# kezakool/flair-for-aigle

Hardware: AMD Instinct MI355X
Metric: 512x512x5 tiles/sec (train fwd+bwd+AdamW), U-Net ResNet-34, 19 classes (higher is better)
Workload: dtype bf16; 1 GPU; synthetic 512x512x5 tiles, 19-class U-Net (ResNet-34 encoder), batch 32 per GPU, train step (BASELINE.json configs[1]); global_batch=32, tile=512, parallelism=dp1

## Files before the change

flair-for-aigle_amd/csrc/conv_igemm.hip:

```cpp
#include "ffa_gfx950.h"

#include <stdlib.h>

#ifndef FFA_CONV_READS_FIRST
#define FFA_CONV_READS_FIRST 0
#endif

#ifndef FFA_CONV_TRACE
#define FFA_CONV_TRACE 0
#endif
#if FFA_CONV_TRACE
#ifndef FFA_CONV_TRACE_FIRST
#define FFA_CONV_TRACE_FIRST 0
#endif
__device__ long long ffa_conv_trace_buf[64 * 256];
#define FFA_TRACE(slot_)                                                                    \
  if (trace_on) {                                                                           \
    if (trace_n < 256) ffa_conv_trace_buf[(blockIdx.x - FFA_CONV_TRACE_FIRST) * 256 + trace_n] = (long long)(slot_) << 56 | (__builtin_readcyclecounter() & 0xFFFFFFFFFFFFFFLL); \
    ++trace_n;                                                                              \
  }
#else
#define FFA_TRACE(slot_)
#endif

// ... 867 lines not shown
            }
            if (res) {
#pragma unroll
              for (int i = 0; i < 4; ++i) v[i] += ffa_load_elem<T>(res + pix + c0 + i);
            }
            if (a.relu) {
#pragma unroll
              for (int i = 0; i < 4; ++i) v[i] = fmaxf(v[i], 0.f);
            }
            if (EB == 2) {
              uint2 u;
              u.x = ffa_pack_bf16x2(v[0], v[1]);
              u.y = ffa_pack_bf16x2(v[2], v[3]);
              *reinterpret_cast<uint2*>(out + pix + c0) = u;
            } else {
              *reinterpret_cast<float4*>(out + pix + c0) = make_float4(v[0], v[1], v[2], v[3]);
            }
            if (want_stats) {
#pragma unroll
              for (int i = 0; i < 4; ++i) {
                const float r = (EB == 2) ? ffa_bf16_bits_to_f32(ffa_f32_to_bf16_bits(v[i])) : v[i];
                st[g * 4 + i] += r;
                st[NCH + g * 4 + i] = __builtin_fmaf(r, r, st[NCH + g * 4 + i]);
              }
            }
          }
        }
      }
      if (want_stats) {
#pragma unroll
        for (int bit = 4; bit >= 0; --bit) {
          const int n = (2 * NCH) >> (4 - bit);
          if (n > 2) {
            const bool up = (rho >> bit) & 1;
#pragma unroll
            for (int jj = 0; jj < NCH; ++jj) {
              if (jj < n / 2) {
                float lo = st[jj], hi = st[jj + n / 2];
                asm volatile("" : "+v"(lo), "+v"(hi));
                const float keep = up ? hi : lo;
                const float send = up ? lo : hi;
                st[jj] = keep + __shfl_xor(send, 1 << bit, 64);
              }
            }
          } else {
            st[0] += __shfl_xor(st[0], 1 << bit, 64);
            st[1] += __shfl_xor(st[1], 1 << bit, 64);
          }
        }
        red[(wpx * 64 + lane) * 2 + 0] = st[0];
        red[(wpx * 64 + lane) * 2 + 1] = st[1];
        __syncthreads();
        constexpr int NOUT = (G::MT == 2) ? 128 : 64;
        if (tid < NOUT) {
          const int jj = tid & 1;
          const int ln = (G::MT == 2) ? (tid >> 1) : ((tid >> 1) * 2);
          float t = 0.f;
#pragma unroll
          for (int w = 0; w < WPX; ++w) t += red[(w * 64 + ln) * 2 + jj];
          const int r5 = ln & 31, hf = ln >> 5;
          const int which = r5 >> 4;
          int c;
          if (G::MT == 2) {
            const int L = (r5 & 15) * 2 + jj;
            c = cur.cb * BCO + 16 * (L >> 3) + 8 * hf + (L & 7);
          } else {
            const int L = ((r5 >> 1) & 7) * 2 + jj;
            c = cur.cb * BCO + 8 * (L >> 2) + 4 * hf + (L & 3);
          }
          if (c < a.Co) a.stats[((size_t)cur.pt * 2 + which) * a.Co + c] = t;
        }
        __syncthreads();
      }
    }
    if (!has_next) break;
    vb = nvb;
    cur = nxt;
    w_b = w_n;
  }
#undef FFA_P_STORE_W
#undef FFA_P_STORE_H
}


struct ConvPlan {
  int bco;
  int rg;
  int th, tw;
};

static int conv_rg(int kh) { return kh == 7 ? 1 : kh; }

static int conv_pref_bco(int kh, int kw, int stride, int cout) {
  if (kh == 3 && kw == 3 && stride == 1) return cout > 32 ? 64 : 32;
  return cout > 32 ? 64 : 32;
}

static bool conv_supported(int kh, int kw, int stride, int bco) {
  const bool shape = (kh == 3 && kw == 3 && (stride == 1 || stride == 2)) ||
                     (kh == 1 && kw == 1 && (stride == 1 || stride == 2)) || (kh == 7 && kw == 7 && stride == 2);
  if (!shape) return false;
  return bco == 64 || bco == 32;
}

static int conv_persist_grid(int dil, int c1_out, const void* bnx, int grid) {
  const char* pe = getenv("FFA_CONV_PERSIST");
  if ((pe && pe[0] == '0') || dil != 1 || c1_out != 0 || bnx != nullptr) return 0;
  const char* pm = getenv("FFA_CONV_PERSIST_MIN");
  const char* pg = getenv("FFA_CONV_PERSIST_GRID");
  const int min_grid = pm ? atoi(pm) : 0;
  int pgrid = pg ? atoi(pg) : 512;
  pgrid = pgrid < 8 ? 8 : (pgrid / 8) * 8;
  if (grid <= min_grid) return 0;
  return pgrid < grid ? pgrid : grid;
}

template <typename T, int KH, int KW, int STRIDE, int RG, int BCO, int WCO, int WPX, int TH, int TW, int HK,
          bool UP = false>
static int launch_hk(const ConvArgs& a, hipStream_t stream) {
  const int grid = ffa_cdiv(a.npt, 8) * 8 * a.ncb;
  if constexpr (KH == 3 && KW == 3 && STRIDE == 1 && HK >= 2 && !UP && WCO == 1 && WPX == 4) {
    const int pgrid = conv_persist_grid(a.dil, a.c1_out, a.bnx, grid);
    if (pgrid > 0) {
      hipLaunchKernelGGL((conv3x3_persist_kernel<T, BCO, TH, TW, HK>), dim3(pgrid), dim3(256), 0, stream, a);
      return ffa_check_launch("conv3x3_persist");
    }
  }
  hipLaunchKernelGGL((conv_igemm_kernel<T, KH, KW, STRIDE, RG, BCO, WCO, WPX, TH, TW, HK, UP>), dim3(grid),
                     dim3(64 * WCO * WPX), 0, stream, a);
  return ffa_check_launch("conv_igemm");
}

template <typename T, int BCO, int TH, int TW>
static int launch_up(const ConvArgs& a, hipStream_t stream) {
  if (a.nchunks % 4 == 0) return launch_hk<T, 3, 3, 1, 3, BCO, 1, 4, TH, TW, 4, true>(a, stream);
  return launch_hk<T, 3, 3, 1, 3, BCO, 1, 4, TH, TW, 2, true>(a, stream);
}

template <typename T, int KH, int KW, int STRIDE, int RG, int BCO, int WCO, int WPX, int TH, int TW>
static int launch_cfg(const ConvArgs& a, hipStream_t stream) {
  if constexpr (KH == 3 && STRIDE == 1) {
    if (a.nchunks % 4 == 0) return launch_hk<T, KH, KW, STRIDE, RG, BCO, WCO, WPX, TH, TW, 4>(a, stream);
    if (a.nchunks % 2 == 0) return launch_hk<T, KH, KW, STRIDE, RG, BCO, WCO, WPX, TH, TW, 2>(a, stream);
  }
  return launch_hk<T, KH, KW, STRIDE, RG, BCO, WCO, WPX, TH, TW, 1>(a, stream);
}

template <typename T, int KH, int KW, int STRIDE, int RG>
static int launch_shape(const ConvArgs& a, const ConvPlan& p, hipStream_t stream) {
  const bool wide = (p.tw == 32);
#define FFA_CONV_CASE(BCO_, WCO_, WPX_)                                                      \
  if (p.bco == BCO_) {                                                                       \
    return wide ? launch_cfg<T, KH, KW, STRIDE, RG, BCO_, WCO_, WPX_, 8, 32>(a, stream)      \
                : launch_cfg<T, KH, KW, STRIDE, RG, BCO_, WCO_, WPX_, 16, 16>(a, stream);    \
  }
  FFA_CONV_CASE(64, 1, 4)
  FFA_CONV_CASE(32, 1, 4)
#undef FFA_CONV_CASE
  ffa_set_error("conv: no kernel for bco=%d", p.bco);
  return FFA_ERR_UNSUPPORTED;
}

template <typename T>
static int launch_dtype(const ConvArgs& a, int kh, int kw, int stride, const ConvPlan& p, hipStream_t stream) {
  if (kh == 3 && kw == 3 && stride == 1) return launch_shape<T, 3, 3, 1, 3>(a, p, stream);
  if (kh == 3 && kw == 3 && stride == 2) return launch_shape<T, 3, 3, 2, 3>(a, p, stream);
// ... 23 lines not shown
      return (cout <= 16 ? 16 : 32) | FFA_BCO_THIN | (ci_pitch == 32 ? FFA_BCO_THIN32 : 0);
  }
  allow_ring &= 1;
  const char* e = getenv("FFA_RING");
  const int eb = (dtype == FFA_BF16) ? 2 : 4;
  const bool on = (dtype == FFA_BF16) ? !(e && e[0] == '0') : (e && e[0] == '1');
  if (allow_ring && on && kh == 3 && kw == 3 && stride == 1 && cout >= 64 && (ci_pitch * eb) % 64 == 0)
    return 64 | FFA_BCO_RING;
  return bco;
}

extern "C" int ffa_conv_row_group(int kh) { return conv_rg(kh); }

static int conv2d_impl(int dtype, const void* in, const void* w_packed, const float* bias, const void* residual,
                       void* out, float* stat_partials, int B, int Hi, int Wi, int Ci, int Ho, int Wo, int Co,
                       int co_rows, int bco, int kh, int kw, int stride, int pad, int dil, int relu,
                       hipStream_t stream, void* out2 = nullptr, int c1_out = 0, const void* bnx = nullptr,
                       const float* bn_sc = nullptr, const float* bn_sh = nullptr) {
  FFA_REQUIRE(dtype == FFA_BF16 || dtype == FFA_F32, "conv: bad dtype %d", dtype);
  FFA_REQUIRE(in && w_packed && out, "conv: null pointer");
  FFA_REQUIRE(B > 0 && Hi > 0 && Wi > 0 && Ho > 0 && Wo > 0, "conv: bad dims");
  FFA_REQUIRE(Ci % 16 == 0 && Co % 8 == 0, "conv: channel pitch must be a multiple of 16 (in) / 8 (out), got %d/%d", Ci, Co);
  FFA_REQUIRE(dil == 1 || dil == 2, "conv: dil must be 1 or 2");
  FFA_REQUIRE(dil == 1 || stride == 1, "conv: zero-insertion input needs stride 1");
  FFA_REQUIRE((long long)B * Hi * Wi * Ci * (dtype == FFA_BF16 ? 2 : 4) < (1LL << 31),
              "conv: input tensor must be smaller than 2 GiB (32-bit piece offsets)");
  if (bco & FFA_BCO_STEM) {
    FFA_REQUIRE(dtype == FFA_BF16 && kh == 7 && kw == 7 && stride == 2 && pad == 3 && dil == 1 && c1_out == 0 && bnx == nullptr &&
                    residual == nullptr,
                "conv: a stem-layout operand serves the bf16 7x7 stride-2 pad-3 convolution only (no residual input)");
    return ffa_stem_conv7x7(in, w_packed, bias, out, stat_partials, B, Hi, Wi, Ci, Ho, Wo, Co, relu, stream);
  }
  if (bco & FFA_BCO_THIN) {
    FFA_REQUIRE(dtype == FFA_BF16 && kh == 3 && kw == 3 && stride == 1 && pad == 1 && dil == 1 && Hi == Ho && Wi == Wo &&
                    bnx == nullptr,
                "conv: a thin-layout operand serves bf16 3x3 stride-1 pad-1 convolutions only");
    if (c1_out > 0) {
      FFA_REQUIRE(c1_out == Co && out2 == nullptr && !stat_partials, "conv: thin pooled form takes C2 = 0 only");
      return ffa_thin_conv3x3(in, w_packed, nullptr, nullptr, out, nullptr, B, Hi, Wi, Ci, Co, co_rows, 0, 0, 1, stream);
    }
    return ffa_thin_conv3x3(in, w_packed, bias, residual, out, stat_partials, B, Hi, Wi, Ci, Co, co_rows, relu, 0, 0,
                            stream);
  }
  if (bco & FFA_BCO_RING) {
    FFA_REQUIRE(kh == 3 && kw == 3 && stride == 1 && pad == 1 && dil == 1 && Hi == Ho && Wi == Wo && c1_out == 0 &&
                    bnx == nullptr,
                "conv: a ring-layout operand serves plain 3x3 stride-1 pad-1 convolutions only");
    return ffa_ring_conv3x3(dtype, in, w_packed, bias, residual, out, stat_partials, nullptr, nullptr, B, Hi, Wi, Ci, Co,
                            co_rows, relu, stream);
  }
  if (!conv_supported(kh, kw, stride, bco)) {
    ffa_set_error("conv: unsupported kernel %dx%d stride %d block %d", kh, kw, stride, bco);
    return FFA_ERR_UNSUPPORTED;
  }
  ConvPlan p;
  p.bco = bco;
  p.rg = conv_rg(kh);
  p.tw = (Wo >= 32) ? 32 : 16;
  p.th = (Wo >= 32) ? 8 : 16;
  FFA_REQUIRE(co_rows % p.bco == 0, "conv: packed weight rows %d not a multiple of block %d", co_rows, p.bco);
  ConvArgs a;
  a.in = in;
  a.w = w_packed;
  a.out = out;
  a.bias = bias;
  a.stats = stat_partials;
  a.in2 = nullptr;
  a.c1_bytes = 0;
  a.out2 = out2;
  a.c1_out = c1_out;
  a.bnx = bnx;
  a.bn_sc = bn_sc;
  a.bn_sh = bn_sh;
  a.res = residual;
  a.B = B; a.Hi = Hi; a.Wi = Wi; a.Ci = Ci;
  a.Ho = Ho; a.Wo = Wo; a.Co = Co;
  a.pad = pad; a.dil = dil; a.relu = relu;
  const int eb = (dtype == FFA_BF16) ? 2 : 4;
  a.nchunks = Ci * eb / 32;
  a.tiles_x = ffa_cdiv(Wo, p.tw);
  a.tiles_y = ffa_cdiv(Ho, p.th);
  a.npt = B * a.tiles_x * a.tiles_y;
  a.ncb = co_rows / p.bco;
  if (dtype == FFA_BF16) return launch_dtype<ffa_bf16>(a, kh, kw, stride, p, stream);
  return launch_dtype<float>(a, kh, kw, stride, p, stream);
}

extern "C" int ffa_conv2d(int dtype, const void* in, const void* w_packed, const float* bias, const void* residual,
                          void* out, int B, int Hi, int Wi, int Ci, int Ho, int Wo, int Co, int co_rows, int bco,
                          int kh, int kw, int stride, int pad, int dil, int relu, hipStream_t stream) {
  return conv2d_impl(dtype, in, w_packed, bias, residual, out, nullptr, B, Hi, Wi, Ci, Ho, Wo, Co, co_rows, bco, kh, kw,
                     stride, pad, dil, relu, stream);
}

extern "C" int ffa_conv2d_pro(int dtype, const void* in, const void* w_packed, const float* bias, const void* residual,
                              void* out, float* stat_partials, const float* pro_scale, const float* pro_shift, int B,
                              int H, int W, int Ci, int Co, int co_rows, int bco, int relu, int up, hipStream_t stream) {
  FFA_REQUIRE(dtype == FFA_BF16 && in && w_packed && out && pro_scale && pro_shift, "conv_pro: bad arguments");
  if (bco & FFA_BCO_THIN)
    return ffa_thin_conv3x3_pro(in, w_packed, bias, residual, out, stat_partials, pro_scale, pro_shift, B, H, W, Ci, Co,
                                co_rows, relu, up, 0, stream);
  if ((bco & FFA_BCO_RING) && !up)
    return ffa_ring_conv3x3(dtype, in, w_packed, bias, residual, out, stat_partials, pro_scale, pro_shift, B, H, W, Ci, Co,
                            co_rows, relu, stream);
  ffa_set_error("conv_pro: no prologue kernel for this operand layout (bco 0x%x, up %d)", bco, up);
  return FFA_ERR_UNSUPPORTED;
}

extern "C" int ffa_conv2d_bnbwd(int dtype, const void* in, const void* w_packed, const void* residual, void* out,
                                float* stat_partials, const void* bnx, const float* bn_scale, const float* bn_shift,
                                int B, int Hi, int Wi, int Ci, int Ho, int Wo, int Co, int co_rows, int bco, int kh,
                                int kw, int stride, int pad, int dil, hipStream_t stream) {
  FFA_REQUIRE(stat_partials && bnx && bn_scale && bn_shift, "conv_bnbwd: null pointer");
  return conv2d_impl(dtype, in, w_packed, nullptr, residual, out, stat_partials, B, Hi, Wi, Ci, Ho, Wo, Co, co_rows,
                     bco, kh, kw, stride, pad, dil, 0, stream, nullptr, 0, bnx, bn_scale, bn_shift);
}

static long long conv_stat_rows_igemm(int B, int Ho, int Wo) {
  const int tw = (Wo >= 32) ? 32 : 16, th = (Wo >= 32) ? 8 : 16;
  return (long long)B * ffa_cdiv(Wo, tw) * ffa_cdiv(Ho, th);
}
extern "C" long long ffa_conv_stat_rows(int B, int Ho, int Wo, int co_rows, int bco) {
  if (bco & FFA_BCO_STEM) return ffa_stem_stat_rows(B, Ho, Wo);
  if (bco & FFA_BCO_THIN) return ffa_thin_stat_rows(B, Ho, Wo, (bco & FFA_BCO_THIN32) ? 32 : 16);
  if (bco & FFA_BCO_RING) return ffa_ring_stat_rows(B, Ho, Wo, co_rows);
  return conv_stat_rows_igemm(B, Ho, Wo);
}

extern "C" int ffa_conv_is_persistent(int dtype, int B, int Ho, int Wo, int Ci, int co_rows, int bco, int kh, int kw,
                                      int stride, int dil) {
  if (!(kh == 3 && kw == 3 && stride == 1) || bco <= 0 || co_rows % bco != 0) return 0;
  const int nchunks = Ci * (dtype == FFA_BF16 ? 2 : 4) / 32;
  if (nchunks % 2 != 0) return 0;
  if (bco & (FFA_BCO_RING | FFA_BCO_THIN | FFA_BCO_STEM)) return 0;
  const int npt = (int)conv_stat_rows_igemm(B, Ho, Wo);
  return conv_persist_grid(dil, 0, nullptr, ffa_cdiv(npt, 8) * 8 * (co_rows / bco)) > 0 ? 1 : 0;
}

extern "C" int ffa_conv2d_stats(int dtype, const void* in, const void* w_packed, const float* bias,
                                const void* residual, void* out, float* stat_partials, int B, int Hi, int Wi, int Ci,
                                int Ho, int Wo, int Co, int co_rows, int bco, int kh, int kw, int stride, int pad,
                                int dil, int relu, hipStream_t stream) {
  FFA_REQUIRE(stat_partials, "conv_stats: null statistics buffer");
  return conv2d_impl(dtype, in, w_packed, bias, residual, out, stat_partials, B, Hi, Wi, Ci, Ho, Wo, Co, co_rows, bco,
                     kh, kw, stride, pad, dil, relu, stream);
}

extern "C" int ffa_conv2d_upcat(int dtype, const void* lo, const void* skip, const void* w_packed, const float* bias,
                                void* out, float* stat_partials, int B, int Hl, int Wl, int C1, int C2, int Co,
                                int co_rows, int bco, int relu, hipStream_t stream) {
  FFA_REQUIRE(dtype == FFA_BF16 || dtype == FFA_F32, "conv_upcat: bad dtype %d", dtype);
  FFA_REQUIRE(lo && w_packed && out && (skip || C2 == 0), "conv_upcat: null pointer");
  FFA_REQUIRE(B > 0 && Hl > 0 && Wl > 0 && C1 > 0 && C2 >= 0 && C1 % 16 == 0 && C2 % 16 == 0 && Co % 8 == 0,
              "conv_upcat: bad dims");
  const int eb = (dtype == FFA_BF16) ? 2 : 4;
  const int Hi = 2 * Hl, Wi = 2 * Wl, Ci = C1 + C2;
  if (bco & FFA_BCO_THIN) {
    if (C2 != 0 || dtype != FFA_BF16) {
      ffa_set_error("conv_upcat: a thin-layout operand takes the skip-less form only");
      return FFA_ERR_UNSUPPORTED;
    }
    return ffa_thin_conv3x3(lo, w_packed, bias, nullptr, out, stat_partials, B, Hi, Wi, C1, Co, co_rows, relu, 1, 0, stream);
  }
  FFA_REQUIRE((long long)B * Hi * Wi * (C1 > C2 ? C1 : C2) * eb < (1LL << 31),
              "conv_upcat: source tensors must be smaller than 2 GiB (32-bit piece offsets)");
  if (!conv_supported(3, 3, 1, bco) || co_rows % bco != 0) {
// ... 72 lines not shown
```

flair-for-aigle_amd/csrc/conv_wgrad.hip:

```cpp
#include "ffa_gfx950.h"

#include <stdlib.h>

#ifndef FFA_WGRAD_TRACE
#define FFA_WGRAD_TRACE 0
#endif
#if FFA_WGRAD_TRACE
__device__ long long ffa_wgrad_trace_buf[64 * 256];
#define FFA_WTRACE(slot_)                                                                   \
  if (trace_on) {                                                                           \
    if (trace_n < 256)                                                                      \
      ffa_wgrad_trace_buf[(blockIdx.y * gridDim.x + blockIdx.x) * 256 + trace_n] =          \
          (long long)(slot_) << 56 | (__builtin_readcyclecounter() & 0xFFFFFFFFFFFFFFLL);    \
    ++trace_n;                                                                              \
  }
#else
#define FFA_WTRACE(slot_)
#endif

struct WgradArgs {
  const void* x;
  const void* dy;
  float* slabs;
  int B, Hi, Wi, Ci;
  int Ho, Wo, Co;
  int pad;
  int tiles_x, tiles_y, npt;
  int ncob, ncib, nsplit;
  const void* x2;
  int C1;
  int CoT, CiT;
  const float* pro_sc;
  const float* pro_sh;
  int ci_real;
};

template <int KH, int KW, int STRIDE, int RG, int WCO, int WCI, int WK, int TH, int TW, int EB>
struct WgradGeom {
  static constexpr int NTHR = 64 * WCO * WCI * WK;
  static constexpr int NPX = TH * TW;
  static constexpr bool ONE = (KH == 1 && KW == 1);
  static constexpr int LS = ONE ? 1 : STRIDE;
  static constexpr int GSTEP = ONE ? STRIDE : 1;
  static constexpr int NRG = KH / RG;
  static constexpr int IH = (TH - 1) * LS + RG;
  static constexpr int IW = (TW - 1) * LS + KW;
  static constexpr int TAPS = RG * KW;
  static constexpr int ROWB = 32 * EB;
  static constexpr int PARTS = ROWB / 16;
  static constexpr int DY_BYTES = WCO * NPX * ROWB;
  static constexpr int IN_BYTES = WCI * IH * IW * ROWB;
  static constexpr int STAGE_BYTES = DY_BYTES + IN_BYTES;
  static constexpr bool MERGE = (WK > 1) && (WCO * WCI == 4 || KH == 7);
  static constexpr int MERGE_BYTES = MERGE ? WCO * WCI * (WK - 1) * TAPS * 16 * 64 * 4 : 0;
  static constexpr int LDS_BYTES = STAGE_BYTES > MERGE_BYTES ? STAGE_BYTES : MERGE_BYTES;
  static constexpr int DY_PIECES = WCO * NPX * PARTS;
  static constexpr int IN_PIECES = WCI * IH * IW * PARTS;
  static constexpr int NDP = (DY_PIECES + NTHR - 1) / NTHR;
  static constexpr int NIP = (IN_PIECES + NTHR - 1) / NTHR;
  static constexpr int KSTEPS = NPX / 16;
  static_assert(TW % 16 == 0, "a 16-pixel k-step must stay inside one tile row");
  static_assert(KSTEPS % WK == 0, "k-steps must divide over the k-split waves");
  static_assert(LDS_BYTES <= 160 * 1024, "LDS budget");
};

template <typename T, int KH, int KW, int STRIDE, int RG, int WCO, int WCI, int WK, int TH, int TW, bool PRO = false>
__global__ void __launch_bounds__(64 * WCO * WCI * WK, (sizeof(T) == 2 ? 2 : 1)) conv_wgrad_kernel(WgradArgs a) {
  constexpr int EB = ElemTraits<T>::kBytes;
  static_assert(!PRO || (EB == 2 && KH == 3 && STRIDE == 1), "the prologue lives in the bf16 3x3 stride-1 path");
  using G = WgradGeom<KH, KW, STRIDE, RG, WCO, WCI, WK, TH, TW, EB>;
  __shared__ __align__(16) unsigned char smem[G::LDS_BYTES];
  unsigned char* sDy = smem;
  unsigned char* sIn = smem + G::DY_BYTES;

  const int tid = threadIdx.x;
#if FFA_WGRAD_TRACE
  const bool trace_on = (threadIdx.x == 0 && blockIdx.y * gridDim.x + blockIdx.x < 64);
  int trace_n = 0;
#endif
  FFA_WTRACE(0)
  const int lane = tid & 63;
  const int wave = tid >> 6;
  const int wk = wave / (WCO * WCI);
  const int wco = (wave / WCI) % WCO, wci = wave % WCI;

  int tb = blockIdx.x;
  const int rg = tb % G::NRG;
  tb /= G::NRG;
  const int cib = tb % a.ncib;
  const int cob = tb / a.ncib;
  const int split = blockIdx.y;
  const int co0 = cob * 32 * WCO;
  const int ci0 = cib * 32 * WCI;

  ffa_f32x16 acc[G::TAPS];
#pragma unroll
  for (int t = 0; t < G::TAPS; ++t)
#pragma unroll
    for (int r = 0; r < 16; ++r) acc[t][r] = 0.f;

  const unsigned char* x_b = static_cast<const unsigned char*>(a.x);
  const unsigned char* dy_b = static_cast<const unsigned char*>(a.dy);
  const bool srcA = a.C1 > 0 && ci0 < a.C1;
  const bool srcB = a.C1 > 0 && !srcA;
  if (srcB) x_b = static_cast<const unsigned char*>(a.x2);
  const int xC = srcA ? a.C1 : (srcB ? a.Ci - a.C1 : a.Ci);
  const int xc0 = srcB ? ci0 - a.C1 : ci0;
  const int xH = srcA ? (a.Hi >> 1) : a.Hi, xW = srcA ? (a.Wi >> 1) : a.Wi;

  const int li = lane & 15;
  const int gsel = (lane >> 4) & 1;
  const int khalf = lane >> 5;
  const unsigned char* dyPlane = sDy + wco * (G::NPX * G::ROWB);
  const unsigned char* inPlane = sIn + wci * (G::IH * G::IW * G::ROWB);

  ffa_u32x4 dreg[G::NDP];
  ffa_u32x4 ireg[G::NIP];
// ... 873 lines not shown
#pragma unroll
          for (int nt = 0; nt < NT; ++nt) {
            const ffa_u32x4 bf = tr2(sS + bBase + ((rr + tp / 3) * G::IW + tp % 3) * G::XB + nt * 32, 4 * G::XB);
#pragma unroll
            for (int mt = 0; mt < MT; ++mt)
              acc[mt][nt][tp] = __builtin_amdgcn_mfma_f32_16x16x32_bf16(__builtin_bit_cast(ffa_bf16x8, af[mt]),
                                                                       __builtin_bit_cast(ffa_bf16x8, bf), acc[mt][nt][tp],
                                                                       0, 0, 0);
          }
        }
      }
      slot = (slot + 1) % G::NSLOT;
    }
  }
  ffa_wait_vm_barrier<0>();

  float* red = reinterpret_cast<float*>(smem);
  constexpr int NACC = MT * NT * 9 * 4;
  auto put = [&](int which) {
    float* dst = red + (size_t)which * NACC * 64 + lane;
    int o = 0;
#pragma unroll
    for (int mt = 0; mt < MT; ++mt)
#pragma unroll
      for (int nt = 0; nt < NT; ++nt)
#pragma unroll
        for (int tp = 0; tp < 9; ++tp)
#pragma unroll
          for (int i = 0; i < 4; ++i) dst[(o++) * 64] = acc[mt][nt][tp][i];
  };
  auto add = [&](int which) {
    const float* src = red + (size_t)which * NACC * 64 + lane;
    int o = 0;
#pragma unroll
    for (int mt = 0; mt < MT; ++mt)
#pragma unroll
      for (int nt = 0; nt < NT; ++nt)
#pragma unroll
        for (int tp = 0; tp < 9; ++tp)
#pragma unroll
          for (int i = 0; i < 4; ++i) acc[mt][nt][tp][i] += src[(o++) * 64];
  };
  if (wave >= 2) put(wave - 2);
  __syncthreads();
  if (wave < 2) add(wave);
  __syncthreads();
  if (wave == 1) put(0);
  __syncthreads();
  if (wave != 0) return;
  add(0);

  float* slab = a.slabs + (size_t)blockIdx.x * a.CoT * 9 * a.CiT;
#pragma unroll
  for (int mt = 0; mt < MT; ++mt)
#pragma unroll
    for (int nt = 0; nt < NT; ++nt)
#pragma unroll
      for (int tp = 0; tp < 9; ++tp)
#pragma unroll
        for (int i = 0; i < 4; ++i) {
          const int co = mt * 16 + 4 * kg + i, ci = nt * 16 + li;
          slab[((size_t)co * 9 + tp) * a.CiT + ci] = acc[mt][nt][tp][i];
        }
}


template <int TW_>
struct Wg64Geom {
  static constexpr int TW = TW_, TH = 256 / TW_, IH = TH + 2, IW = TW + 2;
  static constexpr int RS = 32 / TW;
  static constexpr int XP = IH * IW * 8, YP = TH * TW * 8;
  static constexpr int PIECES = XP + YP;
  static constexpr int NHW = (PIECES + 511) / 512;
  static constexpr int X_BYTES = XP * 16;
  static constexpr int SLOT = PIECES * 16;
  static constexpr int ACC_BYTES = 144 * 64 * 4;
  static constexpr int LDS_BYTES = (2 * SLOT > 4 * ACC_BYTES) ? 2 * SLOT : 4 * ACC_BYTES;
  static_assert(TW == 32 || TW == 16, "tile width");
  static_assert(LDS_BYTES <= 160 * 1024, "LDS budget");
};

__device__ __forceinline__ int wg64_phi(int px) { return ((px >> 1) & 1) | (((px >> 3) & 1) << 1); }

template <int TW>
__global__ void __launch_bounds__(512) conv3x3_wgrad64_kernel(WgradArgs a) {
  using G = Wg64Geom<TW>;
  __shared__ __align__(16) unsigned char smem[G::LDS_BYTES];
  const int tid = threadIdx.x;
  const int lane = tid & 63;
  const int wave = __builtin_amdgcn_readfirstlane(tid >> 6);
  const int kgp = wave >> 2;
  const int wco = (wave >> 1) & 1, wci = wave & 1;
  const int li = lane & 15, kg = lane >> 4;
  const int cib = blockIdx.x % a.ncib, cob = blockIdx.x / a.ncib;
  const int co0 = cob * 64, ci0 = cib * 64;
  const int split = blockIdx.y;

  const bool two = a.C1 > 0;
  const bool from_lo = two && ci0 < a.C1;
  const size_t xpb = (size_t)(!two ? a.Ci : from_lo ? a.C1 : a.Ci - a.C1) * 2, ypb = (size_t)a.Co * 2;
  const int xW = from_lo ? a.Wi / 2 : a.Wi, xH = from_lo ? a.Hi / 2 : a.Hi;
  int pinfo[G::NHW];
#pragma unroll
  for (int k = 0; k < G::NHW; ++k) {
    const int p = tid + k * 512;
    if (p < G::XP) {
      const int q = p >> 3, yy = q / G::IW, xx = q % G::IW, sl = (p & 7) ^ (2 * wg64_phi(xx));
      const int py = from_lo ? ((yy - 1) >> 1) + 1 : yy, px = from_lo ? ((xx - 1) >> 1) + 1 : xx;
      pinfo[k] = ((((py * xW + px) * (int)xpb) >> 4) + sl) << 13 | (yy << 6) | xx;
    } else if (p < G::PIECES) {
      const int q = (p - G::XP) >> 3, yy = q / G::TW, xx = q % G::TW, sl = (p & 7) ^ (2 * wg64_phi(xx));
      pinfo[k] = ((((yy * a.Wo + xx) * (int)ypb) >> 4) + sl) << 13 | (1 << 12) | (yy << 6) | xx;
    } else {
      pinfo[k] = 1 << 11;
    }
  }
  const unsigned char* x_b = (two && !from_lo) ? static_cast<const unsigned char*>(a.x2) + (ci0 - a.C1) * 2
                                               : static_cast<const unsigned char*>(a.x) + ci0 * 2;
  const unsigned char* dy_b = static_cast<const unsigned char*>(a.dy) + co0 * 2;
  const unsigned char* zero = reinterpret_cast<const unsigned char*>(ffa_zero16);
  const bool has_tail = (G::PIECES % 512 == 0) || (wave * 64 + (G::NHW - 1) * 512 < G::PIECES);

  auto tile_origin = [&](int t, int& b, int& oy0, int& ox0) {
    const int tx = t % a.tiles_x;
    const int t2 = t / a.tiles_x;
    oy0 = (t2 % a.tiles_y) * G::TH;
    b = t2 / a.tiles_y;
    ox0 = tx * G::TW;
  };
  auto issue_tile = [&](int t, int slot) {
    int b, oy0, ox0;
    tile_origin(t, b, oy0, ox0);
    const int xoy = from_lo ? (oy0 >> 1) - 1 : oy0 - 1, xox = from_lo ? (ox0 >> 1) - 1 : ox0 - 1;
    const unsigned char* xt = x_b + ((long long)(b * xH + xoy) * xW + xox) * (long long)xpb;
    const unsigned char* yt = dy_b + ((long long)(b * a.Ho + oy0) * a.Wo + ox0) * (long long)ypb;
#pragma unroll
    for (int k = 0; k < G::NHW; ++k) {
      const int info = pinfo[k];
      const int yy = (info >> 6) & 31, xx = info & 63;
      const bool mixed = (k == G::XP / 512) && (G::XP % 512 != 0);
      const bool is_dy = mixed ? (info & (1 << 12)) != 0 : (k * 512 >= G::XP);
      const int oy = yy + (is_dy ? oy0 : oy0 - 1), ox = xx + (is_dy ? ox0 : ox0 - 1);
      const bool valid = (unsigned)oy < (unsigned)a.Ho && (unsigned)ox < (unsigned)a.Wo;
      const unsigned char* src = valid ? (is_dy ? yt : xt) + (size_t)(((unsigned)info >> 13) << 4) : zero;
      const unsigned dst = (unsigned)(size_t)(__attribute__((address_space(3))) void*)(
          smem + slot * G::SLOT + (wave * 64 + k * 512) * 16);
      if (k + 1 < G::NHW || G::PIECES % 512 == 0) {
        ffa_lds_dma16(src, dst);
      } else if (has_tail) {
        if (!(info & (1 << 11))) ffa_lds_dma16(src, dst);
      }
      __builtin_amdgcn_sched_barrier(0);
    }
  };

  ffa_f32x4 acc[2][2][9];
#pragma unroll
  for (int mt = 0; mt < 2; ++mt)
#pragma unroll
    for (int nt = 0; nt < 2; ++nt)
#pragma unroll
      for (int tp = 0; tp < 9; ++tp) acc[mt][nt][tp] = ffa_f32x4{0.f, 0.f, 0.f, 0.f};

  const int kpx = 8 * kg + (li >> 2);
  const int seg = (li & 1) * 8, hbit = (li >> 1) & 1;
  const int yphi = wg64_phi(kpx % G::TW);
  int aoff[2];
#pragma unroll
  for (int mt = 0; mt < 2; ++mt)
    aoff[mt] = G::X_BYTES + (kgp * 128 + kpx) * 128 + (((2 * (wco * 2 + mt) + hbit) ^ (2 * yphi)) * 16) + seg;

  int boff[3][2][2];
#pragma unroll
  for (int sx = 0; sx < 3; ++sx)
#pragma unroll
    for (int nt = 0; nt < 2; ++nt)
#pragma unroll
      for (int h = 0; h < 2; ++h) {
        const int hx = kpx % G::TW + sx + 4 * h;
// ... 346 lines not shown
  p->nsplit = ns;
  const bool merge = p->wk > 1 && (p->wco * p->wci == 4 || stem);
  p->nslab = merge ? ns : ns * p->wk;
  return true;
}

extern "C" long long ffa_conv_wgrad_workspace_bytes(int dtype, int kh, int kw, int stride, int Co, int Ci, int B, int Ho,
                                                    int Wo) {
  WgradPlan p, q;
  if (!wgrad_plan(dtype, kh, kw, stride, Co, Ci, B, Ho, Wo, &p)) return FFA_ERR_UNSUPPORTED;
  long long need = (long long)p.nslab * p.CoT * kh * kw * p.CiT * (long long)sizeof(float);
  if (p.thin) {
    wgrad_plan(dtype, kh, kw, stride, Co, Ci, B, Ho, Wo, &q, true, false);
    const long long other = (long long)q.nslab * q.CoT * kh * kw * q.CiT * (long long)sizeof(float);
    if (other > need) need = other;
  }
  return need;
}

template <typename T, int KH, int KW, int STRIDE, int RG, int WCO, int WCI, int WK, int TH, int TW, bool PRO = false>
static void launch_wgrad_cfg(const WgradArgs& a, int nrg, hipStream_t stream) {
  dim3 grid(a.ncob * a.ncib * nrg, a.nsplit);
  hipLaunchKernelGGL((conv_wgrad_kernel<T, KH, KW, STRIDE, RG, WCO, WCI, WK, TH, TW, PRO>), grid,
                     dim3(64 * WCO * WCI * WK), 0, stream, a);
}

template <typename T>
static int launch_wgrad(const WgradArgs& a, const WgradPlan& p, int kh, int kw, int stride, hipStream_t stream) {
  constexpr bool F32 = (sizeof(T) == 4);
  const bool wide = (p.tw == 32);
  if constexpr (!F32) {
    if (p.thin) {
      const bool up = a.C1 > 0, pro = a.pro_sc != nullptr;
#define FFA_WGTHIN(CI_, CO_)                                                                                     \
  if (a.Ci == CI_ && a.Co == CO_) {                                                                              \
    if (up && pro) hipLaunchKernelGGL((conv3x3_thin_wgrad_kernel<CI_, CO_, true, true>), dim3(a.nsplit), dim3(256), 0, stream, a);   \
    else if (up) hipLaunchKernelGGL((conv3x3_thin_wgrad_kernel<CI_, CO_, true, false>), dim3(a.nsplit), dim3(256), 0, stream, a);    \
    else if (pro) hipLaunchKernelGGL((conv3x3_thin_wgrad_kernel<CI_, CO_, false, true>), dim3(a.nsplit), dim3(256), 0, stream, a);   \
    else hipLaunchKernelGGL((conv3x3_thin_wgrad_kernel<CI_, CO_, false, false>), dim3(a.nsplit), dim3(256), 0, stream, a);           \
    return ffa_check_launch("conv3x3_thin_wgrad");                                                               \
  }
      FFA_WGTHIN(16, 16)
      FFA_WGTHIN(16, 32)
      FFA_WGTHIN(32, 16)
      FFA_WGTHIN(32, 32)
#undef FFA_WGTHIN
      ffa_set_error("conv_wgrad: no thin kernel for pitches %d / %d", a.Ci, a.Co);
      return FFA_ERR_UNSUPPORTED;
    }
    if (p.ring) {
      dim3 grid(a.ncob * a.ncib, a.nsplit);
      if (wide) hipLaunchKernelGGL((conv_wgrad_ring_kernel<4, 32>), grid, dim3(256), 0, stream, a);
      else hipLaunchKernelGGL((conv_wgrad_ring_kernel<8, 16>), grid, dim3(256), 0, stream, a);
      return ffa_check_launch("conv_wgrad_ring");
    }
  }
  if (kh == 3 && stride == 1) {
#define FFA_WG_S1(WCO_, WCI_, WK_, THW_, THN_)                                               \
  if (p.wco == WCO_ && p.wci == WCI_ && p.wk == WK_) {                                       \
    if (wide) launch_wgrad_cfg<T, 3, 3, 1, 3, WCO_, WCI_, WK_, THW_, 32>(a, 1, stream);      \
    else launch_wgrad_cfg<T, 3, 3, 1, 3, WCO_, WCI_, WK_, THN_, 16>(a, 1, stream);           \
    return ffa_check_launch("conv_wgrad");                                                   \
  }
    if constexpr (F32) {
      FFA_WG_S1(2, 1, 1, 4, 8)
      FFA_WG_S1(1, 1, 1, 4, 8)
    } else {
      if (a.pro_sc) {
        if (!(p.wco == 2 && p.wci == 2 && p.wk == 2) || a.C1 > 0) {
          ffa_set_error("conv_wgrad: no prologue for this channel configuration");
          return FFA_ERR_UNSUPPORTED;
        }
        if (wide) launch_wgrad_cfg<T, 3, 3, 1, 3, 2, 2, 2, 8, 32, true>(a, 1, stream);
        else launch_wgrad_cfg<T, 3, 3, 1, 3, 2, 2, 2, 16, 16, true>(a, 1, stream);
        return ffa_check_launch("conv_wgrad");
      }
      {
        const char* e64 = getenv("FFA_WGRAD64");
        const int ih = wide ? 10 : 18, iw = wide ? 34 : 18;
        if (!(e64 && e64[0] == '0') && p.wco == 2 && p.wci == 2 && p.wk == 2 && p.th == (wide ? 8 : 16) && a.C1 % 64 == 0 &&
            (a.C1 == 0 || (a.Hi % 2 == 0 && a.Wi % 2 == 0)) && a.pad == 1 && a.Co % 64 == 0 && a.Ci % 64 == 0 &&
            ((long long)ih * a.Wi + iw) * 2 * (a.Ci > a.Co ? a.Ci : a.Co) < (1LL << 23)) {
          ffa_launch_timed(FFA_KT_WGRAD64, wide ? conv3x3_wgrad64_kernel<32> : conv3x3_wgrad64_kernel<16>,
                           dim3(a.ncob * a.ncib, a.nsplit), dim3(512), stream, a);
          return ffa_check_launch("conv3x3_wgrad64");
        }
      }
      FFA_WG_S1(2, 2, 2, 8, 16)
      FFA_WG_S1(2, 1, 2, 4, 8)
      FFA_WG_S1(1, 2, 2, 4, 8)
      if (p.wco == 1 && p.wci == 1 && p.wk == 4 && (p.th == 8 && wide || p.th == 16 && !wide)) {
        if (wide) launch_wgrad_cfg<T, 3, 3, 1, 3, 1, 1, 4, 8, 32>(a, 1, stream);
        else launch_wgrad_cfg<T, 3, 3, 1, 3, 1, 1, 4, 16, 16>(a, 1, stream);
        return ffa_check_launch("conv_wgrad");
      }
      FFA_WG_S1(1, 1, 4, 4, 8)
    }
#undef FFA_WG_S1
  } else if (kh == 3 && stride == 2) {
    launch_wgrad_cfg<T, 3, 3, 2, 3, 2, F32 ? 1 : 2, 1, 4, 16>(a, 1, stream);
    return ffa_check_launch("conv_wgrad");
  } else if (kh == 1 && stride == 2) {
    launch_wgrad_cfg<T, 1, 1, 2, 1, 2, F32 ? 1 : 2, 1, 4, 16>(a, 1, stream);
    return ffa_check_launch("conv_wgrad");
  } else if (kh == 1 && stride == 1) {
    launch_wgrad_cfg<T, 1, 1, 1, 1, 2, F32 ? 1 : 2, 1, 4, 16>(a, 1, stream);
    return ffa_check_launch("conv_wgrad");
  } else if (kh == 7) {
    if constexpr (!F32) {
      if (p.stem) {
        const char* e8 = getenv("FFA_STEM_WGRAD8");
        if (!(e8 && e8[0] == '0') && a.ci_real <= 8 && a.Ci == 16 && a.Co == 64 && a.pad == 3 && a.Wi <= 3000 && a.Wo <= 1500 &&
            (long long)a.B * a.Hi * a.Wi * 32 < (1LL << 31)) {
          hipLaunchKernelGGL(stem_wgrad8_kernel, dim3(1, a.nsplit), dim3(512), 0, stream, a);
          return ffa_check_launch("stem_wgrad8");
        }
        hipLaunchKernelGGL((stem_wgrad_kernel<0>), dim3(a.Co / 64, a.nsplit), dim3(512), 0, stream, a);
        return ffa_check_launch("stem_wgrad");
      }
    }
    launch_wgrad_cfg<T, 7, 7, 2, 1, 2, 1, F32 ? 1 : 2, 8, 16>(a, 7, stream);
    return ffa_check_launch("conv_wgrad");
  }
  ffa_set_error("conv_wgrad: no kernel for %dx%d stride %d waves %dx%dx%d", kh, kw, stride, p.wco, p.wci, p.wk);
  return FFA_ERR_UNSUPPORTED;
}

static int wgrad_impl(int dtype, const void* x, const void* x2, int C1, const void* dy, float* dw_oihw, int B, int Hi,
                      int Wi, int Ci, int Ho, int Wo, int Co, int Co_real, int Ci_real, int kh, int kw, int stride,
                      int pad, int accumulate, void* workspace, long long workspace_bytes, hipStream_t stream,
                      const float* pro_scale = nullptr, const float* pro_shift = nullptr) {
  FFA_REQUIRE((pro_scale == nullptr) == (pro_shift == nullptr), "conv_wgrad: prologue needs scale and shift");
  FFA_REQUIRE(!pro_scale || (dtype == FFA_BF16 && kh == 3 && kw == 3 && stride == 1 && pad == 1),
              "conv_wgrad: the prologue is for bf16 3x3 stride-1 pad-1 layers");
  FFA_REQUIRE(dtype == FFA_BF16 || dtype == FFA_F32, "conv_wgrad: bad dtype");
  FFA_REQUIRE(x && dy && dw_oihw && workspace, "conv_wgrad: null pointer");
  FFA_REQUIRE(Ci % 8 == 0 && Co % 8 == 0, "conv_wgrad: channel pitch must be a multiple of 8");
  FFA_REQUIRE(Co_real <= Co && Ci_real <= Ci, "conv_wgrad: real channels exceed pitch");
  WgradPlan p;
  const bool thin_ok = pad == 1 && (C1 == 0 || (C1 == Ci && x2 == nullptr));
  if (!wgrad_plan(dtype, kh, kw, stride, Co, Ci, B, Ho, Wo, &p, pad == 1 && C1 == 0, thin_ok)) {
    ffa_set_error("conv_wgrad: unsupported kernel %dx%d stride %d", kh, kw, stride);
    return FFA_ERR_UNSUPPORTED;
  }
  if (C1 > 0 && !p.thin) {
    if (C1 % (32 * p.wci) != 0) {
      ffa_set_error("conv_wgrad_upcat: C1 = %d is not a multiple of the block's %d input channels", C1, 32 * p.wci);
      return FFA_ERR_UNSUPPORTED;
    }
  }
  const long long need = (long long)p.nslab * p.CoT * kh * kw * p.CiT * (long long)sizeof(float);
  if (workspace_bytes < need) {
    ffa_set_error("conv_wgrad: workspace too small (%lld < %lld)", workspace_bytes, need);
    return FFA_ERR_WORKSPACE;
  }
  WgradArgs a;
  a.x = x; a.dy = dy; a.slabs = static_cast<float*>(workspace);
  a.x2 = x2; a.C1 = C1;
  a.pro_sc = pro_scale; a.pro_sh = pro_shift;
  a.ci_real = Ci_real;
  a.B = B; a.Hi = Hi; a.Wi = Wi; a.Ci = Ci;
  a.Ho = Ho; a.Wo = Wo; a.Co = Co;
  a.pad = pad;
  a.tiles_x = p.tiles_x; a.tiles_y = p.tiles_y; a.npt = p.npt;
  a.ncob = p.ncob; a.ncib = p.ncib; a.nsplit = p.nsplit;
  a.CoT = p.CoT; a.CiT = p.CiT;
  int rc = (dtype == FFA_BF16) ? launch_wgrad<ffa_bf16>(a, p, kh, kw, stride, stream)
                               : launch_wgrad<float>(a, p, kh, kw, stride, stream);
  if (rc != FFA_OK) return rc;
  const long long total = (long long)Co_real * kh * kw * ((Ci_real + 3) / 4);
  const char* rv = getenv("FFA_WG_REDUCE_V1");
  const bool reduce_v1 = rv && rv[0] == '1';
  const int cq = (Ci_real + 3) / 4;
  const int v2_blocks = Co_real * ffa_cdiv(cq, p.nslab > 8 ? 8 : 64);
  if (kh == 3 && kw == 3 && !reduce_v1 && v2_blocks >= 512) {
    if (p.nslab > 8) {
      hipLaunchKernelGGL(wgrad_reduce3x3_kernel<32>, dim3(v2_blocks), dim3(256), 0, stream,
                         (const float*)workspace, dw_oihw, p.nslab, p.CoT, p.CiT, Co_real, Ci_real, accumulate);
    } else {
      hipLaunchKernelGGL(wgrad_reduce3x3_kernel<4>, dim3(v2_blocks), dim3(256), 0, stream,
                         (const float*)workspace, dw_oihw, p.nslab, p.CoT, p.CiT, Co_real, Ci_real, accumulate);
    }
    return ffa_check_launch("wgrad_reduce3x3");
  }
  if (p.nslab > 8) {
    long long g = (total + 7) / 8;
    if (g > 4096) g = 4096;
    hipLaunchKernelGGL(wgrad_reduce_kernel<32>, dim3((int)g), dim3(256), 0, stream, (const float*)workspace, dw_oihw,
                       p.nslab, p.CoT, p.CiT, Co_real, Ci_real, kh * kw, accumulate);
  } else {
    long long g = (total + 63) / 64;
    if (g > 4096) g = 4096;
    hipLaunchKernelGGL(wgrad_reduce_kernel<4>, dim3((int)g), dim3(256), 0, stream, (const float*)workspace, dw_oihw,
                       p.nslab, p.CoT, p.CiT, Co_real, Ci_real, kh * kw, accumulate);
  }
  return ffa_check_launch("wgrad_reduce");
}

extern "C" int ffa_conv_wgrad(int dtype, const void* x, const void* dy, float* dw_oihw, int B, int Hi, int Wi, int Ci,
                              int Ho, int Wo, int Co, int Co_real, int Ci_real, int kh, int kw, int stride, int pad,
                              int accumulate, void* workspace, long long workspace_bytes, hipStream_t stream) {
  return wgrad_impl(dtype, x, nullptr, 0, dy, dw_oihw, B, Hi, Wi, Ci, Ho, Wo, Co, Co_real, Ci_real, kh, kw, stride, pad,
                    accumulate, workspace, workspace_bytes, stream);
}

extern "C" int ffa_conv_wgrad_pro(int dtype, const void* x, const void* dy, float* dw_oihw, const float* pro_scale,
                                  const float* pro_shift, int B, int Hi, int Wi, int Ci, int Ho, int Wo, int Co,
                                  int Co_real, int Ci_real, int up, int accumulate, void* workspace,
                                  long long workspace_bytes, hipStream_t stream) {
  FFA_REQUIRE(pro_scale && pro_shift, "conv_wgrad_pro: null prologue vectors");
  return wgrad_impl(dtype, x, nullptr, up ? Ci : 0, dy, dw_oihw, B, Hi, Wi, Ci, Ho, Wo, Co, Co_real, Ci_real, 3, 3, 1, 1,
                    accumulate, workspace, workspace_bytes, stream, pro_scale, pro_shift);
}

extern "C" int ffa_conv_wgrad_upcat(int dtype, const void* lo, const void* skip, const void* dy, float* dw_oihw, int B,
                                    int Hl, int Wl, int C1, int C2, int Co, int Co_real, int accumulate,
                                    void* workspace, long long workspace_bytes, hipStream_t stream) {
  FFA_REQUIRE(lo && (skip || C2 == 0) && C1 > 0 && C2 >= 0, "conv_wgrad_upcat: bad arguments");
  return wgrad_impl(dtype, lo, skip, C1, dy, dw_oihw, B, 2 * Hl, 2 * Wl, C1 + C2, 2 * Hl, 2 * Wl, Co, Co_real, C1 + C2,
                    3, 3, 1, 1, accumulate, workspace, workspace_bytes, stream);
}


__global__ void probe_tr16_kernel(const uint16_t* __restrict__ src, uint16_t* __restrict__ dst) {
  __shared__ __align__(16) unsigned char buf[64 * 128];
  for (int i = threadIdx.x; i < 64 * 64; i += 64) reinterpret_cast<uint16_t*>(buf)[i] = src[i];
  __syncthreads();
  const int lane = threadIdx.x;
  const int li = lane & 15;
  const int grp = lane >> 4;
  const unsigned char* p = buf + (4 * grp + (li >> 2)) * 128 + grp * 32 + (li & 3) * 8;
  ffa_s16x4 v = ffa_lds_read_tr16(p);
#pragma unroll
  for (int e = 0; e < 4; ++e) dst[lane * 4 + e] = (uint16_t)v[e];
}

extern "C" int ffa_probe_tr16(const uint16_t* src, uint16_t* dst, hipStream_t stream) {
  hipLaunchKernelGGL(probe_tr16_kernel, dim3(1), dim3(64), 0, stream, src, dst);
  return ffa_check_launch("probe_tr16");
}

__global__ void probe_mfma_kernel(const float* __restrict__ A, const float* __restrict__ Bm, float* __restrict__ D,
                                  int use_f32) {
// ... 44 lines not shown
```

Measured before the change: 2378 tiles/s.

## Add phase-decomposed dgrad kernel for stride-2 convs and XCD-aware wgrad64 block order

Adds a dedicated kernel for the dilated stride-1 3x3 conv used as the data gradient of a stride-2 conv. It splits the output into four parity classes, so each tap only multiplies the non-zero input samples and the work spent on inserted zeros is skipped. The kernel double-buffers weights and halo in LDS and fuses bias, residual and relu. Separately, the wgrad64 kernel now uses a flattened 1D grid whose block index is remapped so that consecutive logical blocks land on the same XCD, which is meant to improve L2 reuse. Both paths are on by default and can be disabled through environment variables.

Result: no change. 2397 tiles/s (median of 6 runs) (+0.8%).

```diff
diff --git a/flair-for-aigle_amd/csrc/conv_igemm.hip b/flair-for-aigle_amd/csrc/conv_igemm.hip
--- a/flair-for-aigle_amd/csrc/conv_igemm.hip
+++ b/flair-for-aigle_amd/csrc/conv_igemm.hip
@@ -973,6 +973,164 @@
 #undef FFA_P_STORE_H
 }
 
+template <int TH_, int TW_>
+struct DgradS2Geom {
+  static constexpr int TH = TH_, TW = TW_, NTHR = 512, BCO = 64, HK = 4, TAPS = 9;
+  static constexpr int IH = TH + 1, IW = TW + 1;
+  static constexpr int PP = HK * 32 + 16, HPP = 2 * HK;
+  static constexpr int WP = TAPS * 32 + 16;
+  static constexpr int HALO_BYTES = IH * IW * PP, W_BYTES = BCO * WP;
+  static constexpr int LDS_BYTES = 2 * (HALO_BYTES + W_BYTES);
+  static constexpr int W_PIECES = BCO * TAPS * 2, H_PIECES = IH * IW * HPP;
+  static constexpr int NWP = (W_PIECES + NTHR - 1) / NTHR, NHP = (H_PIECES + NTHR - 1) / NTHR;
+  static_assert(TH * TW == 32 * (NTHR / 64), "one 32-position fragment per wave");
+  static_assert(LDS_BYTES <= 160 * 1024, "LDS budget");
+};
+
+template <int TH, int TW>
+__global__ void __launch_bounds__(512) conv_dgrad_s2_kernel(ConvArgs a) {
+  using G = DgradS2Geom<TH, TW>;
+  using T = ffa_bf16;
+  __shared__ __align__(16) unsigned char smem[G::LDS_BYTES];
+  unsigned char* sIn = smem;
+  unsigned char* sW = smem + 2 * G::HALO_BYTES;
+
+  const int bid = blockIdx.x;
+  const int pt = ((bid >> 3) / a.ncb) * 8 + (bid & 7);
+  const int cb = (bid >> 3) % a.ncb;
+  if (pt >= a.npt) return;
+  const int t2 = pt / a.tiles_x;
+  const int b = t2 / a.tiles_y;
+  const int i0 = (t2 % a.tiles_y) * TH, j0 = (pt % a.tiles_x) * TW;
+
+  const int tid = threadIdx.x;
+  const int lane = tid & 63, wave = tid >> 6;
+  const int rho = lane & 31, half = lane >> 5;
+  const int n = wave * 32 + rho;
+  const int py = n / TW, px = n % TW;
+  int aoff[2];
+#pragma unroll
+  for (int mt = 0; mt < 2; ++mt) aoff[mt] = (mt * 32 + rho) * G::WP + half * 16;
+  const int boff = (py * G::IW + px) * G::PP + half * 16;
+
+  ffa_f32x16 acc[4][2];
+#pragma unroll
+  for (int c = 0; c < 4; ++c)
+#pragma unroll
+    for (int mt = 0; mt < 2; ++mt)
+#pragma unroll
+      for (int r = 0; r < 16; ++r) acc[c][mt][r] = 0.f;
+
+  constexpr int SLAB = G::BCO * G::TAPS * 32;
+  const unsigned char* in_b = static_cast<const unsigned char*>(a.in);
+  const unsigned char* w_b = static_cast<const unsigned char*>(a.w) + (size_t)cb * a.nchunks * SLAB;
+
+  int hoff[G::NHP], hlds[G::NHP];
+#pragma unroll
+  for (int k = 0; k < G::NHP; ++k) {
+    const int i = tid + k * G::NTHR;
+    const int q = i / G::HPP, hh = i % G::HPP;
+    const int vy = i0 + q / G::IW, vx = j0 + q % G::IW;
+    const bool ok = i < G::H_PIECES && vy < a.Hi && vx < a.Wi;
+    hoff[k] = ok ? (((b * a.Hi + vy) * a.Wi + vx) * a.Ci * 2 + hh * 16) : -1;
+    hlds[k] = q * G::PP + hh * 16;
+  }
+  ffa_u32x4 wreg[G::NWP], hreg[G::NHP];
+  auto load_w = [&](int c) {
+    const ffa_u32x4* wsrc = reinterpret_cast<const ffa_u32x4*>(w_b + (size_t)c * SLAB);
+#pragma unroll
+    for (int k = 0; k < G::NWP; ++k) {
+      const int i = tid + k * G::NTHR;
+      wreg[k] = wsrc[i < G::W_PIECES ? i : 0];
+    }
+  };
+  auto load_h = [&](int g) {
+    const unsigned char* base = in_b + g * (G::HK * 32);
+#pragma unroll
+    for (int k = 0; k < G::NHP; ++k) {
+      const ffa_u32x4 v = *reinterpret_cast<const ffa_u32x4*>(base + (unsigned)(hoff[k] >= 0 ? hoff[k] : 0));
+      hreg[k] = hoff[k] >= 0 ? v : ffa_u32x4{0u, 0u, 0u, 0u};
+    }
+  };
+  auto store_w = [&](int buf) {
+#pragma unroll
+    for (int k = 0; k < G::NWP; ++k) {
+      const int i = tid + k * G::NTHR;
+      if (i < G::W_PIECES)
+        *reinterpret_cast<ffa_u32x4*>(sW + buf * G::W_BYTES + (i / (G::TAPS * 2)) * G::WP + (i % (G::TAPS * 2)) * 16) = wreg[k];
+    }
+  };
+  auto store_h = [&](int buf) {
+#pragma unroll
+    for (int k = 0; k < G::NHP; ++k)
+      if (tid + k * G::NTHR < G::H_PIECES) *reinterpret_cast<ffa_u32x4*>(sIn + buf * G::HALO_BYTES + hlds[k]) = hreg[k];
+  };
+
+  load_w(0);
+  load_h(0);
+  store_w(0);
+  store_h(0);
+  if (a.nchunks > 1) load_w(1);
+  __syncthreads();
+  for (int c = 0; c < a.nchunks; ++c) {
+    const int g = c / G::HK, j = c % G::HK;
+    if (c + 1 < a.nchunks) store_w((c + 1) & 1);
+    if (c + 2 < a.nchunks) load_w(c + 2);
+    if (j == G::HK - 1 && c + 1 < a.nchunks) store_h((g + 1) & 1);
+    if (j == 0 && c + G::HK < a.nchunks) load_h(g + 1);
+    const unsigned char* sWc = sW + (c & 1) * G::W_BYTES;
+    const unsigned char* sInc = sIn + (g & 1) * G::HALO_BYTES + j * 32;
+#pragma unroll
+    for (int tap = 0; tap < G::TAPS; ++tap) {
+      const int r = tap / 3, s = tap % 3;
+      const int cls = ((r != 1) ? 2 : 0) | ((s != 1) ? 1 : 0);
+      const int shift = ((r == 2) ? G::IW : 0) + ((s == 2) ? 1 : 0);
+      const ffa_u32x4 bf = *reinterpret_cast<const ffa_u32x4*>(sInc + boff + shift * G::PP);
+#pragma unroll
+      for (int mt = 0; mt < 2; ++mt) {
+        const ffa_u32x4 af = *reinterpret_cast<const ffa_u32x4*>(sWc + aoff[mt] + tap * 32);
+        Mma<T>::run(af, bf, acc[cls][mt]);
+      }
+    }
+    __syncthreads();
+  }
+
+  T* out = static_cast<T*>(a.out);
+  const T* res = static_cast<const T*>(a.res);
+#pragma unroll
+  for (int cls = 0; cls < 4; ++cls) {
+    const int oy = 2 * (i0 + py) + (cls >> 1), ox = 2 * (j0 + px) + (cls & 1);
+    if (oy >= a.Ho || ox >= a.Wo) continue;
+    const long long pix = ((long long)(b * a.Ho + oy) * a.Wo + ox) * (long long)a.Co;
+#pragma unroll
+    for (int g = 0; g < 4; ++g) {
+      const int c0 = cb * G::BCO + 16 * g + 8 * half;
+      if (c0 >= a.Co) continue;
+      float v[8];
+#pragma unroll
+      for (int i = 0; i < 4; ++i) {
+        v[i] = acc[cls][0][4 * g + i];
+        v[4 + i] = acc[cls][1][4 * g + i];
+      }
+      if (a.bias) {
+#pragma unroll
+        for (int i = 0; i < 8; ++i) v[i] += a.bias[c0 + i];
+      }
+      if (res) {
+        float rv[8];
+        ffa_load8<T>(res + pix + c0, rv);
+#pragma unroll
+        for (int i = 0; i < 8; ++i) v[i] += rv[i];
+      }
+      if (a.relu) {
+#pragma unroll
+        for (int i = 0; i < 8; ++i) v[i] = fmaxf(v[i], 0.f);
+      }
+      ffa_store8<T>(out + pix + c0, v);
+    }
+  }
+}
+
 
 struct ConvPlan {
   int bco;
@@ -1162,6 +1320,20 @@
   a.tiles_y = ffa_cdiv(Ho, p.th);
   a.npt = B * a.tiles_x * a.tiles_y;
   a.ncb = co_rows / p.bco;
+  {
+    const char* es = getenv("FFA_DGRAD_S2");
+    if (!(es && es[0] == '0') && dtype == FFA_BF16 && dil == 2 && stride == 1 && kh == 3 && kw == 3 && pad == 1 &&
+        p.bco == 64 && !stat_partials && c1_out == 0 && !bnx && a.nchunks % 4 == 0) {
+      const bool wide = Wi >= 32;
+      a.tiles_x = ffa_cdiv((Wo + 1) / 2, wide ? 32 : 16);
+      a.tiles_y = ffa_cdiv((Ho + 1) / 2, wide ? 8 : 16);
+      a.npt = B * a.tiles_x * a.tiles_y;
+      const dim3 grid(ffa_cdiv(a.npt, 8) * 8 * a.ncb);
+      if (wide) hipLaunchKernelGGL((conv_dgrad_s2_kernel<8, 32>), grid, dim3(512), 0, stream, a);
+      else hipLaunchKernelGGL((conv_dgrad_s2_kernel<16, 16>), grid, dim3(512), 0, stream, a);
+      return ffa_check_launch("conv_dgrad_s2");
+    }
+  }
   if (dtype == FFA_BF16) return launch_dtype<ffa_bf16>(a, kh, kw, stride, p, stream);
   return launch_dtype<float>(a, kh, kw, stride, p, stream);
 }
diff --git a/flair-for-aigle_amd/csrc/conv_wgrad.hip b/flair-for-aigle_amd/csrc/conv_wgrad.hip
--- a/flair-for-aigle_amd/csrc/conv_wgrad.hip
+++ b/flair-for-aigle_amd/csrc/conv_wgrad.hip
@@ -33,6 +33,7 @@
   const float* pro_sc;
   const float* pro_sh;
   int ci_real;
+  int xcd_order;
 };
 
 template <int KH, int KW, int STRIDE, int RG, int WCO, int WCI, int WK, int TH, int TW, int EB>
@@ -1072,6 +1073,11 @@
 
 __device__ __forceinline__ int wg64_phi(int px) { return ((px >> 1) & 1) | (((px >> 3) & 1) << 1); }
 
+__device__ __forceinline__ int wg64_decode(int L, int total) {
+  const int k = L & 7, q = total >> 3, r = total & 7;
+  return k * q + (k < r ? k : r) + (L >> 3);
+}
+
 template <int TW>
 __global__ void __launch_bounds__(512) conv3x3_wgrad64_kernel(WgradArgs a) {
   using G = Wg64Geom<TW>;
@@ -1082,9 +1088,11 @@
   const int kgp = wave >> 2;
   const int wco = (wave >> 1) & 1, wci = wave & 1;
   const int li = lane & 15, kg = lane >> 4;
-  const int cib = blockIdx.x % a.ncib, cob = blockIdx.x / a.ncib;
+  const int nblk = a.ncob * a.ncib;
+  const int vb = a.xcd_order ? wg64_decode(blockIdx.x, nblk * a.nsplit) : (int)blockIdx.x;
+  const int split = vb / nblk, blk = vb % nblk;
+  const int cib = blk % a.ncib, cob = blk / a.ncib;
   const int co0 = cob * 64, ci0 = cib * 64;
-  const int split = blockIdx.y;
 
   const bool two = a.C1 > 0;
   const bool from_lo = two && ci0 < a.C1;
@@ -1597,7 +1605,7 @@
             (a.C1 == 0 || (a.Hi % 2 == 0 && a.Wi % 2 == 0)) && a.pad == 1 && a.Co % 64 == 0 && a.Ci % 64 == 0 &&
             ((long long)ih * a.Wi + iw) * 2 * (a.Ci > a.Co ? a.Ci : a.Co) < (1LL << 23)) {
           ffa_launch_timed(FFA_KT_WGRAD64, wide ? conv3x3_wgrad64_kernel<32> : conv3x3_wgrad64_kernel<16>,
-                           dim3(a.ncob * a.ncib, a.nsplit), dim3(512), stream, a);
+                           dim3(a.ncob * a.ncib * a.nsplit), dim3(512), stream, a);
           return ffa_check_launch("conv3x3_wgrad64");
         }
       }
@@ -1674,6 +1682,8 @@
   a.x2 = x2; a.C1 = C1;
   a.pro_sc = pro_scale; a.pro_sh = pro_shift;
   a.ci_real = Ci_real;
+  const char* ex = getenv("FFA_WGRAD64_XCD");
+  a.xcd_order = (ex && ex[0] == '0') ? 0 : 1;
   a.B = B; a.Hi = Hi; a.Wi = Wi; a.Ci = Ci;
   a.Ho = Ho; a.Wo = Wo; a.Co = Co;
   a.pad = pad;
```
